# jmoraispk/DeepMIMO

Hardware: AMD Instinct MI355X
Metric: user-channels/sec (higher is better)
Workload: dtype f16x3-split MFMA, f32 accumulate

## Files before the change

deepmimo_amd/csrc/k2c_beam_power.hip:

```cpp
#include "k2_mfma_frag.h"
#include "dmx_tuning.h"
#include <stdlib.h>

namespace dmx {

static constexpr int BP_SLOT = 16 * 1024;
static constexpr int BP_BUFS = 2;

struct BeamPowArgs {
    int64_t user_begin;
    int m_rx, ue_mh, n_beams;
    int M;
    int K;
    const int32_t* sc;
    double inv_n;
    const float2* ftab;
    const int32_t* fexp;
    float* out;
    int32_t* best;
    int adaptive;
};

__host__ __device__ inline size_t beam_pow_lds_bytes(int M, int NW) {
    const size_t nblk = ((size_t)M + 32 * NW - 1) / (32 * NW);
    return (size_t)BP_BUFS * (NW / 4) * BP_SLOT + LPAD * (8 + 4 + 4) + 16 + nblk * NW * 32 * 4;
}

template <int NW>
__global__ __launch_bounds__(NW * 64, 4) void k2c_beam_power(WsView ws, BeamPowArgs a, int64_t user_count) {
    constexpr int BP_WAVES = NW, BP_CHUNK = NW / 4, MAX_ROWS = 32 * NW;
    extern __shared__ __attribute__((aligned(16))) unsigned char smem[];
    unsigned char* bbuf = smem;
    float* bbuf_f = reinterpret_cast<float*>(smem);
    float2* qtab = reinterpret_cast<float2*>(smem + (size_t)BP_BUFS * BP_CHUNK * BP_SLOT);
    float* crtab = reinterpret_cast<float*>(qtab + LPAD);
    float* citab = crtab + LPAD;
    float* misc = citab + LPAD;
    float* rs = misc + 4;
    const int tid = threadIdx.x, lane = tid & 63;
    const int wave = __builtin_amdgcn_readfirstlane(tid >> 6);
    const int col = lane & 31, hh = lane >> 5;
    const int B = a.n_beams, M = a.M, P = ws.P;
    const int nwide = (a.K + 31) >> 5;
    const int nblk = (M + MAX_ROWS - 1) / MAX_ROWS;

    for (int64_t ul = blockIdx.x; ul < user_count; ul += gridDim.x) {
        const int64_t u = a.user_begin + ul;
        int n_act = ws.n_keep[u];
        n_act = n_act < LPAD ? n_act : LPAD;
        if (n_act == 0) {
            for (int b = tid; b < B; b += BP_WAVES * 64) a.out[(size_t)ul * B + b] = 0.f;
            if (a.best && tid == 0) a.best[ul] = -1;
            continue;
        }
        const size_t rb = (size_t)u * P;
        if (wave == 0) {
            float m = 0.f;
            if (lane < n_act) m = fmaxf(fabsf(ws.c_re[rb + lane]), fabsf(ws.c_im[rb + lane]));
            for (int off = 32; off > 0; off >>= 1) m = fmaxf(m, __shfl_xor(m, off));
            const int l0w = ((n_act - 1) >> 3) << 3;
            float a2 = 0.f;
            if (lane < n_act) a2 = fmaf(ws.c_re[rb + lane], ws.c_re[rb + lane], ws.c_im[rb + lane] * ws.c_im[rb + lane]);
            float m2 = a2, mw2 = lane >= l0w ? a2 : 0.f;
            for (int off = 32; off > 0; off >>= 1) { m2 = fmaxf(m2, __shfl_xor(m2, off)); mw2 = fmaxf(mw2, __shfl_xor(mw2, off)); }
            if (lane == 0) misc[3] = (a.adaptive && l0w >= 8 && mw2 * 4194304.0f <= m2) ? 1.f : 0.f;
            int e;
            (void)frexpf(m, &e);
            const float gs = ldexpf(1.0f, 10 - e);
            if (lane < LPAD) {
                const bool ok = lane < n_act;
                const double q = ok ? (double)ws.dn[rb + lane] * a.inv_n : 0.0;
                const double qh = rint(q * 4096.0) * (1.0 / 4096.0);
                qtab[lane] = make_float2((float)qh, (float)(q - qh));
                crtab[lane] = ok ? ws.c_re[rb + lane] * gs : 0.f;
                citab[lane] = ok ? ws.c_im[rb + lane] * gs : 0.f;
            }
            const int ea = 6 - a.fexp[ul];
            if (lane == 0) { misc[0] = ldexpf(1.0f, e - 10 - ea); misc[1] = ldexpf(1.0f, ea); misc[2] = gs; }
        }
        __syncthreads();
        const float ascale = misc[1];
        const int nfull = ((n_act + 7) >> 3) - (misc[3] != 0.f ? 1 : 0);

        for (int blk = 0; blk < nblk; ++blk) {
            const int row0 = blk * MAX_ROWS;
            const int nrows = (M - row0) < MAX_ROWS ? (M - row0) : MAX_ROWS;
            const int ntiles = (nrows + 31) >> 5;
            const int ntp = ntiles <= 1 ? 1 : (ntiles <= 2 ? 2 : (ntiles <= 4 ? 4 : 8));
            const int tile = wave & (ntp - 1), grp = wave / ntp, ngrp = BP_WAVES / ntp;
            const bool active = tile < ntiles;
            h8 Ah[4], Al[4];
#pragma unroll
            for (int s = 0; s < 4; ++s) { Ah[s] = h8{0, 0, 0, 0, 0, 0, 0, 0}; Al[s] = Ah[s]; }
            if (active) {
                const int r = row0 + (tile << 5) + col;
                const bool pok = r < M;
                const int rx = pok ? r / B : 0, bm = pok ? r - rx * B : 0;
                const double yr = (double)(rx % a.ue_mh), zr = (double)(rx / a.ue_mh);
                const float2* frow = a.ftab + ((size_t)ul * B + bm) * P;
#pragma unroll
                for (int s = 0; s < 4; ++s) {
                    if (8 * s < n_act) {
#pragma unroll
                        for (int jj = 0; jj < 4; ++jj) {
                            const int pl = 8 * s + 4 * hh + jj;
                            h2 vh = {(_Float16)0.f, (_Float16)0.f}, vl = vh;
                            if (pok && pl < n_act) {
                                float sn, cs;
                                sincos_rev(frac_rev(yr * ws.rx_y[rb + pl] + zr * ws.rx_z[rb + pl]), sn, cs);
                                const float2 f = frow[pl];
                                split2_f16((cs * f.x - sn * f.y) * ascale, (cs * f.y + sn * f.x) * ascale, vh, vl, ws.neg_one);
                            }
                            Ah[s][2 * jj] = vh[0]; Ah[s][2 * jj + 1] = vh[1];
                            Al[s][2 * jj] = vl[0]; Al[s][2 * jj + 1] = vl[1];
                        }
                    }
                }
            }
            typedef float pv2 __attribute__((ext_vector_type(2)));
            pv2 rowsum[8];
#pragma unroll
            for (int i = 0; i < 8; ++i) rowsum[i] = pv2{0.f, 0.f};

            auto generate = [&](int c0, int buf) {
                const int wsi = c0 + (wave >> 2), st = wave & 3;
                const int kidx = (wsi << 5) + col;
                const bool kok = wsi < nwide && kidx < a.K;
                const int kki = kok ? a.sc[kidx] : 0;
                const float kl = (float)(kki & 4095), kf = (float)kki;
                h8* slot = reinterpret_cast<h8*>(bbuf + (size_t)(buf * BP_CHUNK + (wave >> 2)) * BP_SLOT);
                h8 rh = h8{0, 0, 0, 0, 0, 0, 0, 0}, rl = rh, ih = rh, il = rh;
                if (kok && 8 * st < n_act) {
#pragma unroll
                    for (int jj = 0; jj < 4; ++jj) {
                        const int pl = 8 * st + 4 * hh + jj;
                        const float2 q = qtab[pl];
                        const float p1 = q.x * kl;
                        float sn, cs;
                        sincos_rev(fmaf(q.y, kf, p1 - rintf(p1)), sn, cs);
                        const float cr = crtab[pl], ci = citab[pl];
                        h2 vh, vl;
                        split2_f16(cr * cs + ci * sn, ci * cs - cr * sn, vh, vl, ws.neg_one);
                        const unsigned hb = __builtin_bit_cast(unsigned, vh), lb = __builtin_bit_cast(unsigned, vl);
                        const h2 reh = __builtin_bit_cast(h2, hb ^ 0x80000000u), rel = __builtin_bit_cast(h2, lb ^ 0x80000000u);
                        const h2 imh = __builtin_bit_cast(h2, __builtin_amdgcn_alignbit(hb, hb, 16));
                        const h2 iml = __builtin_bit_cast(h2, __builtin_amdgcn_alignbit(lb, lb, 16));
                        rh[2 * jj] = reh[0]; rh[2 * jj + 1] = reh[1]; rl[2 * jj] = rel[0]; rl[2 * jj + 1] = rel[1];
                        ih[2 * jj] = imh[0]; ih[2 * jj + 1] = imh[1]; il[2 * jj] = iml[0]; il[2 * jj + 1] = iml[1];
                    }
                }
                slot[(4 * st + 0) * 64 + lane] = rh;
                slot[(4 * st + 1) * 64 + lane] = rl;
                slot[(4 * st + 2) * 64 + lane] = ih;
                slot[(4 * st + 3) * 64 + lane] = il;
            };
            __syncthreads();
            generate(0, 0);
            __syncthreads();
            int buf = 0;
            for (int c0 = 0; c0 < nwide; c0 += BP_CHUNK, buf ^= 1) {
                if (c0 + BP_CHUNK < nwide) generate(c0 + BP_CHUNK, buf ^ 1);
                if (active) {
                    for (int j = grp; j < BP_CHUNK && c0 + j < nwide; j += ngrp) {
                        const h8* slot = reinterpret_cast<const h8*>(bbuf + (size_t)(buf * BP_CHUNK + j) * BP_SLOT);
                        f16v are, aim;
#pragma unroll
                        for (int i = 0; i < 16; ++i) { are[i] = 0.f; aim[i] = 0.f; }
#pragma unroll
                        for (int s = 0; s < 4; ++s) {
                            if (8 * s < n_act) {
                                const h8 rh = slot[(4 * s + 0) * 64 + lane], rl = slot[(4 * s + 1) * 64 + lane];
                                const h8 ih = slot[(4 * s + 2) * 64 + lane], il = slot[(4 * s + 3) * 64 + lane];
                                are = __builtin_amdgcn_mfma_f32_32x32x16_f16(Ah[s], rh, are, 0, 0, 0);
                                aim = __builtin_amdgcn_mfma_f32_32x32x16_f16(Ah[s], ih, aim, 0, 0, 0);
                                if (s >= nfull) continue;
                                are = __builtin_amdgcn_mfma_f32_32x32x16_f16(Ah[s], rl, are, 0, 0, 0);
                                aim = __builtin_amdgcn_mfma_f32_32x32x16_f16(Ah[s], il, aim, 0, 0, 0);
                                are = __builtin_amdgcn_mfma_f32_32x32x16_f16(Al[s], rh, are, 0, 0, 0);
                                aim = __builtin_amdgcn_mfma_f32_32x32x16_f16(Al[s], ih, aim, 0, 0, 0);
                            }
                        }
                        DMX_MFMA_RESULT_GUARD2(are, aim);
#pragma unroll
                        for (int i = 0; i < 8; ++i) {
                            const pv2 re = {are[2 * i], are[2 * i + 1]}, im = {aim[2 * i], aim[2 * i + 1]};
                            const pv2 p = __builtin_elementwise_fma(re, re, im * im);
                            rowsum[i] += pv2{__builtin_amdgcn_sqrtf(p.x), __builtin_amdgcn_sqrtf(p.y)};
                        }
                    }
                }
                __syncthreads();
            }
            if (active) {
#pragma unroll
                for (int i = 0; i < 16; ++i) {
                    float v = (i & 1) ? rowsum[i >> 1].y : rowsum[i >> 1].x;
                    for (int off = 16; off > 0; off >>= 1) v += __shfl_xor(v, off);
                    if (col == 0) rs[((blk * BP_WAVES + wave) << 5) + (i & 3) + 8 * (i >> 2) + 4 * hh] = v;
                }
            }
        }
        __syncthreads();
        const float norm = misc[0] / ((float)a.m_rx * (float)a.K);
        for (int b = tid; b < B; b += BP_WAVES * 64) {
            float t = 0.f;
            for (int rx = 0; rx < a.m_rx; ++rx) {
                const int r = rx * B + b, blk = r / MAX_ROWS, w = r - blk * MAX_ROWS, tile = w >> 5;
                const int nrows = (M - blk * MAX_ROWS) < MAX_ROWS ? (M - blk * MAX_ROWS) : MAX_ROWS;
                const int ntiles = (nrows + 31) >> 5;
                const int ntp = ntiles <= 1 ? 1 : (ntiles <= 2 ? 2 : (ntiles <= 4 ? 4 : 8));
                for (int g = 0; g < BP_WAVES / ntp; ++g) t += rs[((blk * BP_WAVES + g * ntp + tile) << 5) + (w & 31)];
            }
            t *= norm;
            a.out[(size_t)ul * B + b] = t;
            bbuf_f[b] = t;
        }
        __syncthreads();
        if (a.best && tid == 0) {
            int arg = 0;
            float mx = bbuf_f[0];
            for (int b = 1; b < B; ++b) { if (bbuf_f[b] > mx) { mx = bbuf_f[b]; arg = b; } }
            a.best[ul] = arg;
        }
        __syncthreads();
    }
}

int launch_beam_power(const dmx_params& prm, const WsView& ws, int64_t user_begin, int64_t user_count,
                      const float2* codebook, int n_beams, void* beam_ws, float* out_amp, int32_t* out_best, hipStream_t stream) {
    if (user_count == 0 || n_beams == 0) return DMX_OK;
    BeamPowArgs a;
    a.user_begin = user_begin;
    a.m_rx = prm.ue_shape[0] * prm.ue_shape[1];
    a.ue_mh = prm.ue_shape[0];
    a.n_beams = n_beams;
    a.M = a.m_rx * n_beams;
    const int nw = tuning_int("DMX_BEAM_WAVES", 8) == 4 ? 4 : 8;
    const size_t smem = beam_pow_lds_bytes(a.M, nw);
    if (smem > 160 * 1024) { set_error("%d x %d (rx, beam) rows are too many for the beam-power kernel", a.m_rx, n_beams); return DMX_ERR_SHAPE; }
    BeamTabs t;
    int rc = launch_beam_project(prm, ws, user_begin, user_count, codebook, n_beams, beam_ws, stream, &t);
    if (rc) return rc;
    a.K = prm.n_selected;
    a.sc = prm.selected_subcarriers;
    a.inv_n = 1.0 / (double)prm.n_subcarriers;
    a.ftab = t.ftab;
    a.fexp = t.fexp;
    a.out = out_amp;
    a.best = out_best;
    a.adaptive = (prm.flags & DMX_FLAG_ADAPTIVE_TERMS) ? 1 : 0;
    const auto kernel = nw == 4 ? k2c_beam_power<4> : k2c_beam_power<8>;
    int64_t grid = resident_workgroups(kernel, nw * 64, smem);
    const int64_t g4 = user_count / 4;
    if (g4 > grid) grid = g4 < 4 * grid ? g4 : 4 * grid;
    if (grid > user_count) grid = user_count;
    return launch_dyn_lds(kernel, "k2c_beam_power", dim3((unsigned)grid), dim3(nw * 64), smem, smem, stream, ws, a, user_count);
}

}
```

Baseline: 6.506 million.

## Specialize beam-power kernel on path-slab count and tail mode, pack small tails

Templates the row-block loop on the number of active 8-path slabs and a tail mode (full, weak, packed), dispatched through a uniform switch. MFMA passes and LDS slot writes for unused slabs and low-part tails are dropped at compile time, and tails of one or two paths are packed into a single fragment. Other changes: gains are prefetched into registers before the n_keep check, the row-sum reductions use DPP adds, and the best-beam argmax becomes a wave-parallel reduction. The cost is more template instantiations and code size, plus register-pressure risk, and the packed tail layout has to match the MFMA operand mapping to stay correct.

```diff
diff --git a/deepmimo_amd/csrc/k2c_beam_power.hip b/deepmimo_amd/csrc/k2c_beam_power.hip
--- a/deepmimo_amd/csrc/k2c_beam_power.hip
+++ b/deepmimo_amd/csrc/k2c_beam_power.hip
@@ -6,6 +6,9 @@
 
 static constexpr int BP_SLOT = 16 * 1024;
 static constexpr int BP_BUFS = 2;
+
+static constexpr int BP_TAIL_FULL = 0, BP_TAIL_WEAK = 1, BP_TAIL_PACK = 2;
+template <int V> struct BpInt { static constexpr int value = V; };
 
 struct BeamPowArgs {
     int64_t user_begin;
@@ -26,6 +29,18 @@
     return (size_t)BP_BUFS * (NW / 4) * BP_SLOT + LPAD * (8 + 4 + 4) + 16 + nblk * NW * 32 * 4;
 }
 
+template <int CTRL>
+__device__ __forceinline__ float dpp_add(float v) {
+    const int x = __builtin_bit_cast(int, v);
+    return v + __builtin_bit_cast(float, __builtin_amdgcn_update_dpp(x, x, CTRL, 0xf, 0xf, false));
+}
+
+__device__ __forceinline__ int hidden_tid() {
+    int t = threadIdx.x;
+    asm volatile("" : "+v"(t));
+    return t;
+}
+
 template <int NW>
 __global__ __launch_bounds__(NW * 64, 4) void k2c_beam_power(WsView ws, BeamPowArgs a, int64_t user_count) {
     constexpr int BP_WAVES = NW, BP_CHUNK = NW / 4, MAX_ROWS = 32 * NW;
@@ -37,15 +52,18 @@
     float* citab = crtab + LPAD;
     float* misc = citab + LPAD;
     float* rs = misc + 4;
-    const int tid = threadIdx.x, lane = tid & 63;
-    const int wave = __builtin_amdgcn_readfirstlane(tid >> 6);
-    const int col = lane & 31, hh = lane >> 5;
+    const int wave = __builtin_amdgcn_readfirstlane(threadIdx.x >> 6);
     const int B = a.n_beams, M = a.M, P = ws.P;
     const int nwide = (a.K + 31) >> 5;
     const int nblk = (M + MAX_ROWS - 1) / MAX_ROWS;
 
     for (int64_t ul = blockIdx.x; ul < user_count; ul += gridDim.x) {
+        const int tid = hidden_tid();
+        const int lane = tid & 63;
         const int64_t u = a.user_begin + ul;
+        const size_t rb = (size_t)u * P;
+        float rec_re = 0.f, rec_im = 0.f, rec_dn = 0.f;
+        if (wave == 0 && lane < LPAD && lane < P) { rec_re = ws.c_re[rb + lane]; rec_im = ws.c_im[rb + lane]; rec_dn = ws.dn[rb + lane]; }
         int n_act = ws.n_keep[u];
         n_act = n_act < LPAD ? n_act : LPAD;
         if (n_act == 0) {
@@ -53,87 +71,104 @@
             if (a.best && tid == 0) a.best[ul] = -1;
             continue;
         }
-        const size_t rb = (size_t)u * P;
+        const int l0w = ((n_act - 1) >> 3) << 3;
         if (wave == 0) {
-            float m = 0.f;
-            if (lane < n_act) m = fmaxf(fabsf(ws.c_re[rb + lane]), fabsf(ws.c_im[rb + lane]));
-            for (int off = 32; off > 0; off >>= 1) m = fmaxf(m, __shfl_xor(m, off));
-            const int l0w = ((n_act - 1) >> 3) << 3;
-            float a2 = 0.f;
-            if (lane < n_act) a2 = fmaf(ws.c_re[rb + lane], ws.c_re[rb + lane], ws.c_im[rb + lane] * ws.c_im[rb + lane]);
-            float m2 = a2, mw2 = lane >= l0w ? a2 : 0.f;
-            for (int off = 32; off > 0; off >>= 1) { m2 = fmaxf(m2, __shfl_xor(m2, off)); mw2 = fmaxf(mw2, __shfl_xor(mw2, off)); }
+            const bool ok = lane < n_act;
+            const float cre = ok ? rec_re : 0.f, cim = ok ? rec_im : 0.f;
+            const float a2 = fmaf(cre, cre, cim * cim);
+            float m = fmaxf(fabsf(cre), fabsf(cim)), m2 = a2, mw2 = lane >= l0w ? a2 : 0.f;
+            for (int off = 16; off > 0; off >>= 1) {
+                m = fmaxf(m, __shfl_xor(m, off)); m2 = fmaxf(m2, __shfl_xor(m2, off)); mw2 = fmaxf(mw2, __shfl_xor(mw2, off));
+            }
             if (lane == 0) misc[3] = (a.adaptive && l0w >= 8 && mw2 * 4194304.0f <= m2) ? 1.f : 0.f;
             int e;
             (void)frexpf(m, &e);
             const float gs = ldexpf(1.0f, 10 - e);
             if (lane < LPAD) {
-                const bool ok = lane < n_act;
-                const double q = ok ? (double)ws.dn[rb + lane] * a.inv_n : 0.0;
+                const double q = ok ? (double)rec_dn * a.inv_n : 0.0;
                 const double qh = rint(q * 4096.0) * (1.0 / 4096.0);
                 qtab[lane] = make_float2((float)qh, (float)(q - qh));
-                crtab[lane] = ok ? ws.c_re[rb + lane] * gs : 0.f;
-                citab[lane] = ok ? ws.c_im[rb + lane] * gs : 0.f;
+                crtab[lane] = cre * gs;
+                citab[lane] = cim * gs;
             }
             const int ea = 6 - a.fexp[ul];
             if (lane == 0) { misc[0] = ldexpf(1.0f, e - 10 - ea); misc[1] = ldexpf(1.0f, ea); misc[2] = gs; }
         }
         __syncthreads();
         const float ascale = misc[1];
-        const int nfull = ((n_act + 7) >> 3) - (misc[3] != 0.f ? 1 : 0);
-
-        for (int blk = 0; blk < nblk; ++blk) {
-            const int row0 = blk * MAX_ROWS;
-            const int nrows = (M - row0) < MAX_ROWS ? (M - row0) : MAX_ROWS;
-            const int ntiles = (nrows + 31) >> 5;
-            const int ntp = ntiles <= 1 ? 1 : (ntiles <= 2 ? 2 : (ntiles <= 4 ? 4 : 8));
-            const int tile = wave & (ntp - 1), grp = wave / ntp, ngrp = BP_WAVES / ntp;
-            const bool active = tile < ntiles;
-            h8 Ah[4], Al[4];
-#pragma unroll
-            for (int s = 0; s < 4; ++s) { Ah[s] = h8{0, 0, 0, 0, 0, 0, 0, 0}; Al[s] = Ah[s]; }
-            if (active) {
-                const int r = row0 + (tile << 5) + col;
-                const bool pok = r < M;
-                const int rx = pok ? r / B : 0, bm = pok ? r - rx * B : 0;
-                const double yr = (double)(rx % a.ue_mh), zr = (double)(rx / a.ue_mh);
-                const float2* frow = a.ftab + ((size_t)ul * B + bm) * P;
-#pragma unroll
-                for (int s = 0; s < 4; ++s) {
-                    if (8 * s < n_act) {
-#pragma unroll
-                        for (int jj = 0; jj < 4; ++jj) {
-                            const int pl = 8 * s + 4 * hh + jj;
-                            h2 vh = {(_Float16)0.f, (_Float16)0.f}, vl = vh;
-                            if (pok && pl < n_act) {
-                                float sn, cs;
-                                sincos_rev(frac_rev(yr * ws.rx_y[rb + pl] + zr * ws.rx_z[rb + pl]), sn, cs);
-                                const float2 f = frow[pl];
-                                split2_f16((cs * f.x - sn * f.y) * ascale, (cs * f.y + sn * f.x) * ascale, vh, vl, ws.neg_one);
+        const bool weak = misc[3] != 0.f;
+        const bool pack = !weak && n_act - l0w <= 2;
+        const int kind = __builtin_amdgcn_readfirstlane(3 * ((n_act - 1) >> 3) + (weak ? BP_TAIL_WEAK : (pack ? BP_TAIL_PACK : BP_TAIL_FULL)));
+
+        auto row_blocks = [&](auto ns_c, auto tail_c) {
+            constexpr int NS = decltype(ns_c)::value, TAIL = decltype(tail_c)::value;
+            constexpr int NF = TAIL == BP_TAIL_FULL ? NS : NS - 1;
+            for (int blk = 0; blk < nblk; ++blk) {
+                const int lane = hidden_tid() & 63, col = lane & 31, hh = lane >> 5;
+                int Bd = B, mhd = a.ue_mh;
+                asm volatile("" : "+s"(Bd), "+s"(mhd));
+                const int row0 = blk * MAX_ROWS;
+                const int nrows = (M - row0) < MAX_ROWS ? (M - row0) : MAX_ROWS;
+                const int ntiles = (nrows + 31) >> 5;
+                const int ntp = ntiles <= 1 ? 1 : (ntiles <= 2 ? 2 : (ntiles <= 4 ? 4 : 8));
+                const int tile = wave & (ntp - 1), grp = wave / ntp, ngrp = BP_WAVES / ntp;
+                const bool active = tile < ntiles;
+                h8 Ah[NS], Al[NF > 0 ? NF : 1];
+#pragma unroll
+                for (int s = 0; s < NS; ++s) Ah[s] = h8{0, 0, 0, 0, 0, 0, 0, 0};
+#pragma unroll
+                for (int s = 0; s < NF; ++s) Al[s] = h8{0, 0, 0, 0, 0, 0, 0, 0};
+                if (active) {
+                    const int r = row0 + (tile << 5) + col;
+                    const bool pok = r < M;
+                    const int rx = pok ? r / Bd : 0, bm = pok ? r - rx * Bd : 0;
+                    const double yr = (double)(rx % mhd), zr = (double)(rx / mhd);
+                    const float2* frow = a.ftab + ((size_t)ul * B + bm) * P;
+                    auto a_split = [&](int pl, h2& vh, h2& vl) {
+                        vh = h2{(_Float16)0.f, (_Float16)0.f}; vl = vh;
+                        if (pok && pl < n_act) {
+                            float sn, cs;
+                            sincos_rev(frac_rev(yr * ws.rx_y[rb + pl] + zr * ws.rx_z[rb + pl]), sn, cs);
+                            const float2 f = frow[pl];
+                            split2_f16((cs * f.x - sn * f.y) * ascale, (cs * f.y + sn * f.x) * ascale, vh, vl, ws.neg_one);
+                        }
+                    };
+#pragma unroll
+                    for (int s = 0; s < NS; ++s) {
+                        if (TAIL == BP_TAIL_PACK && s == NS - 1) {
+                            h2 vh0, vl0, vh1, vl1;
+                            a_split(8 * s, vh0, vl0);
+                            a_split(8 * s + 1, vh1, vl1);
+                            const h8 lo = {vh0[0], vh0[1], vh1[0], vh1[1], vh0[0], vh0[1], vh1[0], vh1[1]};
+                            const h8 up = {vl0[0], vl0[1], vl1[0], vl1[1], 0, 0, 0, 0};
+                            Ah[s] = hh ? up : lo;
+                        } else {
+#pragma unroll
+                            for (int jj = 0; jj < 4; ++jj) {
+                                h2 vh, vl;
+                                a_split(8 * s + 4 * hh + jj, vh, vl);
+                                Ah[s][2 * jj] = vh[0]; Ah[s][2 * jj + 1] = vh[1];
+                                if (s < NF) { Al[s][2 * jj] = vl[0]; Al[s][2 * jj + 1] = vl[1]; }
                             }
-                            Ah[s][2 * jj] = vh[0]; Ah[s][2 * jj + 1] = vh[1];
-                            Al[s][2 * jj] = vl[0]; Al[s][2 * jj + 1] = vl[1];
                         }
                     }
                 }
-            }
-            typedef float pv2 __attribute__((ext_vector_type(2)));
-            pv2 rowsum[8];
-#pragma unroll
-            for (int i = 0; i < 8; ++i) rowsum[i] = pv2{0.f, 0.f};
-
-            auto generate = [&](int c0, int buf) {
-                const int wsi = c0 + (wave >> 2), st = wave & 3;
-                const int kidx = (wsi << 5) + col;
-                const bool kok = wsi < nwide && kidx < a.K;
-                const int kki = kok ? a.sc[kidx] : 0;
-                const float kl = (float)(kki & 4095), kf = (float)kki;
-                h8* slot = reinterpret_cast<h8*>(bbuf + (size_t)(buf * BP_CHUNK + (wave >> 2)) * BP_SLOT);
-                h8 rh = h8{0, 0, 0, 0, 0, 0, 0, 0}, rl = rh, ih = rh, il = rh;
-                if (kok && 8 * st < n_act) {
-#pragma unroll
-                    for (int jj = 0; jj < 4; ++jj) {
-                        const int pl = 8 * st + 4 * hh + jj;
+                typedef float pv2 __attribute__((ext_vector_type(2)));
+                pv2 rowsum[8];
+#pragma unroll
+                for (int i = 0; i < 8; ++i) rowsum[i] = pv2{0.f, 0.f};
+
+                auto generate = [&](int c0, int buf) {
+                    const int wsi = c0 + (wave >> 2), st = wave & 3;
+                    if (st >= NS) return;
+                    const int lane = hidden_tid() & 63, col = lane & 31, hh = lane >> 5;
+                    const bool last = st == NS - 1;
+                    const int kidx = (wsi << 5) + col;
+                    const bool kok = wsi < nwide && kidx < a.K;
+                    const int kki = kok ? a.sc[kidx] : 0;
+                    const float kl = (float)(kki & 4095), kf = (float)kki;
+                    h8* slot = reinterpret_cast<h8*>(bbuf + (size_t)(buf * BP_CHUNK + (wave >> 2)) * BP_SLOT);
+                    auto g_split = [&](int pl, unsigned& hb, unsigned& lb) {
                         const float2 q = qtab[pl];
                         const float p1 = q.x * kl;
                         float sn, cs;
@@ -141,68 +176,106 @@
                         const float cr = crtab[pl], ci = citab[pl];
                         h2 vh, vl;
                         split2_f16(cr * cs + ci * sn, ci * cs - cr * sn, vh, vl, ws.neg_one);
-                        const unsigned hb = __builtin_bit_cast(unsigned, vh), lb = __builtin_bit_cast(unsigned, vl);
-                        const h2 reh = __builtin_bit_cast(h2, hb ^ 0x80000000u), rel = __builtin_bit_cast(h2, lb ^ 0x80000000u);
-                        const h2 imh = __builtin_bit_cast(h2, __builtin_amdgcn_alignbit(hb, hb, 16));
-                        const h2 iml = __builtin_bit_cast(h2, __builtin_amdgcn_alignbit(lb, lb, 16));
-                        rh[2 * jj] = reh[0]; rh[2 * jj + 1] = reh[1]; rl[2 * jj] = rel[0]; rl[2 * jj + 1] = rel[1];
-                        ih[2 * jj] = imh[0]; ih[2 * jj + 1] = imh[1]; il[2 * jj] = iml[0]; il[2 * jj + 1] = iml[1];
-                    }
-                }
-                slot[(4 * st + 0) * 64 + lane] = rh;
-                slot[(4 * st + 1) * 64 + lane] = rl;
-                slot[(4 * st + 2) * 64 + lane] = ih;
-                slot[(4 * st + 3) * 64 + lane] = il;
-            };
-            __syncthreads();
-            generate(0, 0);
-            __syncthreads();
-            int buf = 0;
-            for (int c0 = 0; c0 < nwide; c0 += BP_CHUNK, buf ^= 1) {
-                if (c0 + BP_CHUNK < nwide) generate(c0 + BP_CHUNK, buf ^ 1);
-                if (active) {
-                    for (int j = grp; j < BP_CHUNK && c0 + j < nwide; j += ngrp) {
-                        const h8* slot = reinterpret_cast<const h8*>(bbuf + (size_t)(buf * BP_CHUNK + j) * BP_SLOT);
-                        f16v are, aim;
-#pragma unroll
-                        for (int i = 0; i < 16; ++i) { are[i] = 0.f; aim[i] = 0.f; }
-#pragma unroll
-                        for (int s = 0; s < 4; ++s) {
-                            if (8 * s < n_act) {
-                                const h8 rh = slot[(4 * s + 0) * 64 + lane], rl = slot[(4 * s + 1) * 64 + lane];
-                                const h8 ih = slot[(4 * s + 2) * 64 + lane], il = slot[(4 * s + 3) * 64 + lane];
+                        hb = __builtin_bit_cast(unsigned, vh); lb = __builtin_bit_cast(unsigned, vl);
+                    };
+                    typedef unsigned u4v __attribute__((ext_vector_type(4)));
+                    u4v rh = {0u, 0u, 0u, 0u}, rl = rh, ih = rh, il = rh;
+                    if (TAIL == BP_TAIL_PACK && last) {
+                        if (kok) {
+#pragma unroll
+                            for (int jj = 0; jj < 2; ++jj) {
+                                unsigned hb = 0u, lb = 0u;
+                                if (8 * st + jj < n_act) g_split(8 * st + jj, hb, lb);
+                                lb = hh ? 0u : lb;
+                                rh[jj] = hb ^ 0x80000000u; rh[2 + jj] = lb ^ 0x80000000u;
+                                ih[jj] = __builtin_amdgcn_alignbit(hb, hb, 16); ih[2 + jj] = __builtin_amdgcn_alignbit(lb, lb, 16);
+                            }
+                        }
+                    } else if (kok) {
+#pragma unroll
+                        for (int jj = 0; jj < 4; ++jj) {
+                            unsigned hb, lb;
+                            g_split(8 * st + 4 * hh + jj, hb, lb);
+                            rh[jj] = hb ^ 0x80000000u; rl[jj] = lb ^ 0x80000000u;
+                            ih[jj] = __builtin_amdgcn_alignbit(hb, hb, 16); il[jj] = __builtin_amdgcn_alignbit(lb, lb, 16);
+                        }
+                    }
+                    slot[(4 * st + 0) * 64 + lane] = __builtin_bit_cast(h8, rh);
+                    slot[(4 * st + 2) * 64 + lane] = __builtin_bit_cast(h8, ih);
+                    if (TAIL == BP_TAIL_FULL || !last) {
+                        slot[(4 * st + 1) * 64 + lane] = __builtin_bit_cast(h8, rl);
+                        slot[(4 * st + 3) * 64 + lane] = __builtin_bit_cast(h8, il);
+                    }
+                };
+                __syncthreads();
+                generate(0, 0);
+                __syncthreads();
+                int buf = 0;
+                for (int c0 = 0; c0 < nwide; c0 += BP_CHUNK, buf ^= 1) {
+                    if (c0 + BP_CHUNK < nwide) generate(c0 + BP_CHUNK, buf ^ 1);
+                    if (active) {
+                        for (int j = grp; j < BP_CHUNK && c0 + j < nwide; j += ngrp) {
+                            const h8* slot = reinterpret_cast<const h8*>(bbuf + (size_t)(buf * BP_CHUNK + j) * BP_SLOT);
+                            f16v are, aim;
+#pragma unroll
+                            for (int i = 0; i < 16; ++i) { are[i] = 0.f; aim[i] = 0.f; }
+#pragma unroll
+                            for (int s = 0; s < NS; ++s) {
+                                const h8 rh = slot[(4 * s + 0) * 64 + lane], ih = slot[(4 * s + 2) * 64 + lane];
                                 are = __builtin_amdgcn_mfma_f32_32x32x16_f16(Ah[s], rh, are, 0, 0, 0);
                                 aim = __builtin_amdgcn_mfma_f32_32x32x16_f16(Ah[s], ih, aim, 0, 0, 0);
-                                if (s >= nfull) continue;
-                                are = __builtin_amdgcn_mfma_f32_32x32x16_f16(Ah[s], rl, are, 0, 0, 0);
-                                aim = __builtin_amdgcn_mfma_f32_32x32x16_f16(Ah[s], il, aim, 0, 0, 0);
-                                are = __builtin_amdgcn_mfma_f32_32x32x16_f16(Al[s], rh, are, 0, 0, 0);
-                                aim = __builtin_amdgcn_mfma_f32_32x32x16_f16(Al[s], ih, aim, 0, 0, 0);
+                                if (s < NF) {
+                                    const h8 rl = slot[(4 * s + 1) * 64 + lane], il = slot[(4 * s + 3) * 64 + lane];
+                                    are = __builtin_amdgcn_mfma_f32_32x32x16_f16(Ah[s], rl, are, 0, 0, 0);
+                                    aim = __builtin_amdgcn_mfma_f32_32x32x16_f16(Ah[s], il, aim, 0, 0, 0);
+                                    are = __builtin_amdgcn_mfma_f32_32x32x16_f16(Al[s], rh, are, 0, 0, 0);
+                                    aim = __builtin_amdgcn_mfma_f32_32x32x16_f16(Al[s], ih, aim, 0, 0, 0);
+                                }
                             }
-                        }
-                        DMX_MFMA_RESULT_GUARD2(are, aim);
-#pragma unroll
-                        for (int i = 0; i < 8; ++i) {
-                            const pv2 re = {are[2 * i], are[2 * i + 1]}, im = {aim[2 * i], aim[2 * i + 1]};
-                            const pv2 p = __builtin_elementwise_fma(re, re, im * im);
-                            rowsum[i] += pv2{__builtin_amdgcn_sqrtf(p.x), __builtin_amdgcn_sqrtf(p.y)};
-                        }
-                    }
+                            DMX_MFMA_RESULT_GUARD2(are, aim);
+#pragma unroll
+                            for (int i = 0; i < 8; ++i) {
+                                const pv2 re = {are[2 * i], are[2 * i + 1]}, im = {aim[2 * i], aim[2 * i + 1]};
+                                const pv2 p = __builtin_elementwise_fma(re, re, im * im);
+                                rowsum[i] += pv2{__builtin_amdgcn_sqrtf(p.x), __builtin_amdgcn_sqrtf(p.y)};
+                            }
+                        }
+                    }
+                    __syncthreads();
                 }
-                __syncthreads();
-            }
-            if (active) {
-#pragma unroll
-                for (int i = 0; i < 16; ++i) {
-                    float v = (i & 1) ? rowsum[i >> 1].y : rowsum[i >> 1].x;
-                    for (int off = 16; off > 0; off >>= 1) v += __shfl_xor(v, off);
-                    if (col == 0) rs[((blk * BP_WAVES + wave) << 5) + (i & 3) + 8 * (i >> 2) + 4 * hh] = v;
+                if (active) {
+                    float v[16];
+#pragma unroll
+                    for (int i = 0; i < 16; ++i) {
+                        const float x = (i & 1) ? rowsum[i >> 1].y : rowsum[i >> 1].x;
+                        v[i] = dpp_add<0x140>(dpp_add<0x141>(dpp_add<0x4e>(dpp_add<0xb1>(x))));
+                    }
+#pragma unroll
+                    for (int i = 0; i < 16; ++i) v[i] += __shfl_xor(v[i], 16);
+#pragma unroll
+                    for (int i = 0; i < 16; ++i)
+                        if (col == 0) rs[((blk * BP_WAVES + wave) << 5) + (i & 3) + 8 * (i >> 2) + 4 * hh] = v[i];
                 }
             }
+        };
+        switch (kind) {
+            case 0: row_blocks(BpInt<1>{}, BpInt<BP_TAIL_FULL>{}); break;
+            case 2: row_blocks(BpInt<1>{}, BpInt<BP_TAIL_PACK>{}); break;
+            case 3: row_blocks(BpInt<2>{}, BpInt<BP_TAIL_FULL>{}); break;
+            case 4: row_blocks(BpInt<2>{}, BpInt<BP_TAIL_WEAK>{}); break;
+            case 5: row_blocks(BpInt<2>{}, BpInt<BP_TAIL_PACK>{}); break;
+            case 6: row_blocks(BpInt<3>{}, BpInt<BP_TAIL_FULL>{}); break;
+            case 7: row_blocks(BpInt<3>{}, BpInt<BP_TAIL_WEAK>{}); break;
+            case 8: row_blocks(BpInt<3>{}, BpInt<BP_TAIL_PACK>{}); break;
+            case 9: row_blocks(BpInt<4>{}, BpInt<BP_TAIL_FULL>{}); break;
+            case 10: row_blocks(BpInt<4>{}, BpInt<BP_TAIL_WEAK>{}); break;
+            default: row_blocks(BpInt<4>{}, BpInt<BP_TAIL_PACK>{}); break;
         }
         __syncthreads();
-        const float norm = misc[0] / ((float)a.m_rx * (float)a.K);
-        for (int b = tid; b < B; b += BP_WAVES * 64) {
+        int Kd = a.K;
+        asm volatile("" : "+s"(Kd));
+        const float norm = misc[0] / ((float)a.m_rx * (float)Kd);
+        for (int b = hidden_tid(); b < B; b += BP_WAVES * 64) {
             float t = 0.f;
             for (int rx = 0; rx < a.m_rx; ++rx) {
                 const int r = rx * B + b, blk = r / MAX_ROWS, w = r - blk * MAX_ROWS, tile = w >> 5;
@@ -216,11 +289,17 @@
             bbuf_f[b] = t;
         }
         __syncthreads();
-        if (a.best && tid == 0) {
-            int arg = 0;
-            float mx = bbuf_f[0];
-            for (int b = 1; b < B; ++b) { if (bbuf_f[b] > mx) { mx = bbuf_f[b]; arg = b; } }
-            a.best[ul] = arg;
+        if (a.best && wave == 0) {
+            const int lane = hidden_tid() & 63;
+            float mx = lane == 0 ? bbuf_f[0] : -INFINITY;
+            int arg = lane == 0 ? 0 : 0x7fffffff;
+            for (int b = lane == 0 ? 64 : lane; b < B; b += 64) { const float t = bbuf_f[b]; if (t > mx) { mx = t; arg = b; } }
+            for (int off = 32; off > 0; off >>= 1) {
+                const float om = __shfl_down(mx, off);
+                const int oa = __shfl_down(arg, off);
+                if (om > mx || (om == mx && oa < arg)) { mx = om; arg = oa; }
+            }
+            if (lane == 0) a.best[ul] = arg;
         }
         __syncthreads();
     }
```

New measurement: 6.503 million. No clear change (-0.0%).
